# RuyiLian/CheckerPose

Hardware: AMD Instinct MI355X
Metric: crops/sec forward (256x256, npt=512) (higher is better)
Workload: dtype bf16; 1 GPU; LMO 'ape' hr18GNN2_res6_gnn3Skip_mlpQuery npt=512, PoseNet_GNNskip forward, deterministic random-init weights; global_batch=256, parallelism=dp1 (no forward collective), launch=hipGraph replay of 104 kernel launches

## Files before the change

### checkerpose_amd/_abi.py

```python
import ctypes as C
import os

_HERE = os.path.dirname(os.path.abspath(__file__))
LIB_PATH = os.environ.get("CHECKERPOSE_AMD_LIB") or os.path.join(_HERE, "libcheckerpose_hip.so")

CP_F32, CP_BF16, CP_F16 = 0, 1, 2
ACT_NONE, ACT_RELU, ACT_LEAKY = 0, 1, 2
LOSS_BCE, LOSS_L1 = 0, 1
POSE_ERR_ADD, POSE_ERR_ADI = 1, 2
BOP_ERR_MSSD, BOP_ERR_MSPD, BOP_ERR_PROJ, BOP_MAP_SMALL, BOP_MAP_LARGE = 1, 2, 4, 16, 32


class CpConvDesc(C.Structure):
    _fields_ = [("dtype", C.c_int32), ("out_f32", C.c_int32), ("B", C.c_int32), ("H", C.c_int32), ("W", C.c_int32),
                ("Cin", C.c_int32), ("in_cstride", C.c_int32), ("in_coff", C.c_int32),
                ("R", C.c_int32), ("S", C.c_int32), ("stride", C.c_int32), ("pad", C.c_int32),
                ("Ho", C.c_int32), ("Wo", C.c_int32), ("Cout", C.c_int32), ("act", C.c_int32), ("slope", C.c_float), ("ksplit", C.c_int32),
                ("o_base", C.c_int64), ("o_sb", C.c_int64), ("o_sy", C.c_int64), ("o_sx", C.c_int64),
                ("o_sc", C.c_int64)]


_P, _I, _F, _L = C.c_void_p, C.c_int, C.c_float, C.c_longlong


# ... 62 lines not shown
                ("Cin", C.c_int32), ("x_cstride", C.c_int32), ("x_coff", C.c_int32),
                ("R", C.c_int32), ("S", C.c_int32), ("stride", C.c_int32), ("pad", C.c_int32),
                ("dw_base", C.c_int64), ("dw_sco", C.c_int64), ("dw_sci", C.c_int64), ("dw_sr", C.c_int64),
                ("dw_ss", C.c_int64)]


SIGNATURES = {
    "cp_version": (_I, []),
    "cp_device_status": (_I, [_P, _I]),
    "cp_set_deterministic": (None, [_I]),
    "cp_get_deterministic": (_I, []),
    "cp_strerror": (C.c_char_p, [_I]),
    "cp_last_kernel": (C.c_char_p, []),
    "cp_kernel_log_begin": (None, []),
    "cp_kernel_log": (C.c_char_p, []),
    "cp_chan_align": (_I, [_I]),
    "cp_packed_weight_bytes": (C.c_size_t, [_I, _I, _I, _I, _I]),
    "cp_pack_conv_weight": (_I, [_P, _I, _P, _I, _I, _I, _I, _I, _I, _I, _P, _I, _P]),
    "cp_conv2d_igemm": (_I, [_P, C.POINTER(CpConvDesc), _P, _P, _P, _P, _P, _P]),
    "cp_conv2d_igemm_splitk": (_I, [_I, C.c_longlong, _I, _I]),
    "cp_packed_halo_weight_bytes": (C.c_size_t, [_I, _I, _I]),
    "cp_pack_conv3x3_halo_weight": (_I, [_P, _I, _P, _I, _I, _I, _P]),
    "cp_conv3x3_halo": (_I, [_P, C.POINTER(CpConvDesc), _P, _P, _P, _P, _P, _P]),
    "cp_conv2x2_halo_supported": (_I, [_I, _I, _I, _I]),
    "cp_packed_conv2x2_halo_weight_bytes": (C.c_size_t, [_I, _I, _I]),
    "cp_pack_conv2x2_halo_weight": (_I, [_P, _I, _P, _I, _I, _I, _P]),
    "cp_conv2x2_halo": (_I, [_P, C.POINTER(CpConvDesc), _P, _P, _P, _P, _P, _P]),
    "cp_conv3x3_s2_small_supported": (_I, [_I, _I, _I, _I]),
    "cp_conv3x3_s2_small_weight_bytes": (C.c_size_t, [_I, _I]),
    "cp_pack_conv3x3_s2_small_weight": (_I, [_P, _P, _I, _I, _I, _I, _P]),
    "cp_conv3x3_s2_small": (_I, [_P, C.POINTER(CpConvDesc), _P, _P, _P, _P, _P]),
    "cp_conv3x3_halo_up2x_supported": (_I, [_I, _I]),
    "cp_conv3x3_halo_up2x": (_I, [_P, C.POINTER(CpConvDesc), _P, _P, _P, _P, _P]),
    "cp_conv3x3_halo_seg_supported": (_I, [_I, _I, _I]),
    "cp_conv3x3_halo_seg": (_I, [_P, C.POINTER(CpConvDesc), _P, _P, _P, _P, _P, _P, _P, _I, _P]),
    "cp_pack_conv3x3_rows_weight": (_I, [_P, _I, _P, _I, _I, _I, _P]),
    "cp_basicblock_fused": (_I, [_P, C.POINTER(CpConvDesc), _P, _P, _P, _P, _P, _P, _P, _P]),
    "cp_bottleneck_fused": (_I, [_P, C.POINTER(CpConvDesc)] + [_P] * 14),
    "cp_packed_gemm_weight_bytes": (C.c_size_t, [_I, _I, _I]),
    "cp_pack_gemm_weight": (_I, [_P, _I, _P, _I, _I, _I, _P]),
    "cp_gemm_rows": (_I, [_P, C.POINTER(CpConvDesc), _P, _P, _P, _P, _P, _P]),
    "cp_mlp_query_fused_supported": (_I, [_I, _I, _I, _I]),
    "cp_mlp_query_fused": (_I, [_P, _P, _I, _I, _I, _I, _P, _P, _P, _F, _P, _P, _P, _F, _P, _P, _P, _L, _L, _L, _L]),
    "cp_mlp_query_fused_t": (_I, [_P, _I, _P, _I, _I, _I, _I, _P, _P, _P, _F, _P, _P, _P, _F, _P, _P, _P, _L, _L, _L, _L]),
    "cp_mlp_query_fused_n": (_I, [_P, _I, _P, _I, _I, _I, _I, _P, _P, _P, _F, _P, _P, _P, _F, _P, _P, _I, _P, _L, _L, _L, _L,
                                  _P, _P, _P, _P]),
    "cp_mlp_pair_fused_supported": (_I, [_I, _I, _I]),
    "cp_mlp_pair_fused": (_I, [_P, _P, _I, _I, _I, _I, _I, _P, _P, _F, _P, _P, _F, _P, _I, _I]),
    "cp_mlp_pair_fused_t": (_I, [_P, _I, _P, _I, _I, _I, _I, _I, _P, _P, _F, _P, _P, _F, _P, _I, _I]),
    "cp_mlp_pair_fused_gather_supported": (_I, [_I, _I, _I]),
    "cp_mlp_pair_fused_gather": (_I, [_P, C.POINTER(CpI2fGather), _P, _I, _I, _I, _I, _I, _P, _P, _F, _P, _P, _F, _P, _I, _I]),
    "cp_mlp_pair_fused_gather_t": (_I, [_P, _I, C.POINTER(CpI2fGather), _P, _I, _I, _I, _I, _I, _P, _P, _F, _P, _P, _F, _P, _I, _I]),
    "cp_hr_stem_weight_bytes": (C.c_size_t, [_I]),
    "cp_pack_hr_stem_weights": (_I, [_P, _P, _P, _P, _P]),
    "cp_hr_stem": (_I, [_P, _P, _I, _I, _I, _P, _P, _P, _P, _P, _P, _P]),
    "cp_hr_chain_supported": (_I, [_I, _I, _I]),
    "cp_hr_chain_weight_bytes": (C.c_size_t, [_I, _I, _I]),
    "cp_hr_chain_affine_floats": (_I, [_I, _I, _I]),
    "cp_pack_hr_chain_weight": (_I, [_P, _P, _P, _I, _I, _I, _I, _P]),
    "cp_hr_branch_chain": (_I, [_P, _I, _I, _I, _I, _I, C.POINTER(_P), C.POINTER(C.c_int32), _I, _P, _P, _P]),
    "cp_hr_chain_tail_supported": (_I, [_I, _I, _I]),
    "cp_hr_chain_tail_weight_bytes": (C.c_size_t, []),
    "cp_hr_chain_tail_channels": (_I, []),
    "cp_pack_hr_chain_tail_weight": (_I, [_P, _P, _P, _I, _I, _I, _P]),
    "cp_hr_branch_chain_tail": (_I, [_P, _I, _I, _I, _I, _I, C.POINTER(_P), C.POINTER(C.c_int32), _I, _P, _P, _P, C.POINTER(CpChainTail)]),
    "cp_hr_chain_tailconv_supported": (_I, [_I, _I, _I, _I, _I]),
# ... 175 lines not shown
```

### checkerpose_amd/engine.py

```python
import ctypes as C
import os

import torch

from . import _abi
from ._abi import ACT_LEAKY, ACT_NONE, ACT_RELU, CP_BF16, CP_F16, CP_F32, CpChainTail, CpChainTailConv, CpConvDesc, CpFuseConv

_TORCH_DT = {CP_F32: torch.float32, CP_BF16: torch.bfloat16}
USE_HALO = os.environ.get("CHECKERPOSE_AMD_HALO", "1") != "0"
USE_FUSED_BN = os.environ.get("CHECKERPOSE_AMD_FUSED_BN", "1") != "0"
USE_FUSED_BB = os.environ.get("CHECKERPOSE_AMD_FUSED_BB", "1") != "0"
USE_GEMM = os.environ.get("CHECKERPOSE_AMD_GEMM", "1") != "0"
USE_CHAIN = os.environ.get("CHECKERPOSE_AMD_CHAIN", "1") != "0"
USE_UP_FUSED = os.environ.get("CHECKERPOSE_AMD_UP_FUSED", "1") != "0"
USE_FUSE_OUT = os.environ.get("CHECKERPOSE_AMD_FUSE_OUT", "1") != "0"
USE_S2_SMALL = os.environ.get("CHECKERPOSE_AMD_S2_SMALL", "1") != "0"
USE_SEG_FUSED = os.environ.get("CHECKERPOSE_AMD_SEG_FUSED", "1") != "0"
USE_HALO2 = os.environ.get("CHECKERPOSE_AMD_HALO2", "1") != "0"
USE_CHAIN_TAILS = os.environ.get("CHECKERPOSE_AMD_CHAIN_TAILS", "1") != "0"
USE_CHAIN_TAIL = os.environ.get("CHECKERPOSE_AMD_CHAIN_TAIL", "1") != "0"
FUSE_OUT_MIN_BATCH = int(os.environ.get("CHECKERPOSE_AMD_FUSE_OUT_MIN_BATCH", "1"))
USE_MLP_FUSED = os.environ.get("CHECKERPOSE_AMD_MLP_FUSED", "1") != "0"
MLP_FUSED_MIN_ROWS = int(os.environ.get("CHECKERPOSE_AMD_MLP_FUSED_MIN_ROWS", "1"))
EDGE_SCHED = os.environ.get("CHECKERPOSE_AMD_EDGE_SCHED", "1") != "0"
USE_SPLITK = os.environ.get("CHECKERPOSE_AMD_SPLITK", "1") != "0"
GEMM_WS_SMALL_K = os.environ.get("CHECKERPOSE_AMD_GEMM_WS_SMALL_K", "1") != "0"
USE_MLP_GATHER = os.environ.get("CHECKERPOSE_AMD_MLP_GATHER", "1") != "0"
USE_PATCH_GATHER = os.environ.get("CHECKERPOSE_AMD_PATCH_GATHER", "1") != "0"
USE_STEM = os.environ.get("CHECKERPOSE_AMD_STEM", "1") != "0"
STEM_MIN_BATCH = int(os.environ.get("CHECKERPOSE_AMD_STEM_MIN_BATCH", "96"))
USE_EDGE_FUSED = os.environ.get("CHECKERPOSE_AMD_EDGE_FUSED", "1") != "0"
USE_GNN_F16 = os.environ.get("CHECKERPOSE_AMD_GNN_F16", "1") != "0"
USE_EDGE_TILED = os.environ.get("CHECKERPOSE_AMD_EDGE_TILED", "1") != "0"
EDGE_FUSED_MIN_BATCH = int(os.environ.get("CHECKERPOSE_AMD_EDGE_FUSED_MIN_BATCH", "96"))
CHAIN_MIN_BATCH = int(os.environ.get("CHECKERPOSE_AMD_CHAIN_MIN_BATCH", "40"))
NO_RECYCLE = os.environ.get("CHECKERPOSE_AMD_NO_RECYCLE", "0") == "1"
DTYPES = {"fp32": CP_F32, "f32": CP_F32, "float32": CP_F32, "bf16": CP_BF16, "bfloat16": CP_BF16}


class _ConvLog(list):

    def __init__(self, prog):
        super().__init__()
        self.prog, self.op_index = prog, []

    def append(self, e):
        super().append(e)
# ... 36 lines not shown
            raise RuntimeError("parameter %s must be an fp32 tensor on %s" % (key, self.device))
        return t.detach().contiguous()

    def pack(self, name, w, Cout, Cin, R, S, cin_phys, cout_rows, transposed=0, phase=0, row_map=None, dtype=None):
        dtype = self.dtype if dtype is None else dtype
        ck = (name, cin_phys, cout_rows, transposed, phase) + (() if dtype == self.dtype else (dtype,))
        if ck in self.cache:
            return self.cache[ck]
        nbytes = self.lib.cp_packed_weight_bytes(dtype, cout_rows, cin_phys, R, S)
        out = torch.empty(nbytes, dtype=torch.uint8, device=self.device)
        rm = None
        if row_map is not None:
            rm = torch.tensor(row_map, dtype=torch.int32, device=self.device)
            self.keep.append(rm)
        w = w.contiguous()
        self.keep.append(w)
        st = torch.cuda.current_stream(self.device).cuda_stream
        _abi.check(self.lib.cp_pack_conv_weight(st, dtype, w.data_ptr(), Cout, Cin, R, S, cin_phys, transposed, phase,
                                                rm.data_ptr() if rm is not None else None, cout_rows, out.data_ptr()),
                   "cp_pack_conv_weight(%s)" % name)
        self.cache[ck] = out
        return out

    def pack_halo(self, name, w, Cout, Cin, cin_phys):
        ck = ("halo", name, cin_phys)
        if ck in self.cache:
            return self.cache[ck]
        out = torch.empty(self.lib.cp_packed_halo_weight_bytes(self.dtype, Cout, cin_phys), dtype=torch.uint8, device=self.device)
        w = w.contiguous()
        self.keep.append(w)
        st = torch.cuda.current_stream(self.device).cuda_stream
        _abi.check(self.lib.cp_pack_conv3x3_halo_weight(st, self.dtype, w.data_ptr(), Cout, Cin, cin_phys, out.data_ptr()),
                   "cp_pack_conv3x3_halo_weight(%s)" % name)
        self.cache[ck] = out
        return out

    def pack_rows3x3(self, name, w, Cout, Cin, cin_phys):
        ck = ("rows3x3", name, cin_phys)
        if ck in self.cache:
            return self.cache[ck]
        out = torch.empty(self.lib.cp_packed_halo_weight_bytes(self.dtype, Cout, cin_phys), dtype=torch.uint8, device=self.device)
        w = w.contiguous()
        self.keep.append(w)
        st = torch.cuda.current_stream(self.device).cuda_stream
        _abi.check(self.lib.cp_pack_conv3x3_rows_weight(st, self.dtype, w.data_ptr(), Cout, Cin, cin_phys, out.data_ptr()),
                   "cp_pack_conv3x3_rows_weight(%s)" % name)
        self.cache[ck] = out
        return out

    def pack_gemm(self, name, w, Cout, Cin, cin_phys, dtype=None):
        dtype = self.dtype if dtype is None else dtype
        ck = ("gemm", name, cin_phys) + (() if dtype == self.dtype else (dtype,))
        if ck in self.cache:
            return self.cache[ck]
        out = torch.empty(self.lib.cp_packed_gemm_weight_bytes(dtype, Cout, cin_phys), dtype=torch.uint8, device=self.device)
        w = w.contiguous()
        self.keep.append(w)
        st = torch.cuda.current_stream(self.device).cuda_stream
        _abi.check(self.lib.cp_pack_gemm_weight(st, dtype, w.data_ptr(), Cout, Cin, cin_phys, out.data_ptr()),
                   "cp_pack_gemm_weight(%s)" % name)
        self.cache[ck] = out
        return out

    def pack_chain(self, name, ws, affs, C_, H, W):
        ck = ("chain", name)
        if ck in self.cache:
# ... 241 lines not shown

    def can_conv_up2x(self, H, W, Cout):
        return (USE_UP_FUSED and 2 * H >= 8 and 2 * W >= 16 and
                bool(self.lib.cp_conv3x3_halo_up2x_supported(self.dtype, _rup(Cout, self.E))))

    def conv_up2x(self, x: Act, wkey, w, scale, shift, act=ACT_NONE, slope=0.0, out: Act = None):
        wCout, wCin = w.shape[0], w.shape[1]
        if wCin != x.C:
            raise RuntimeError("conv %s: weight expects %d input channels, activation has %d" % (wkey, wCin, x.C))
        packed = self.ws.pack_halo(wkey, w, wCout, wCin, x.Cphys)
        sc, sh = self.ws.affine(wkey + "#0", scale, shift, wCout)
        Ho, Wo = 2 * x.H, 2 * x.W
        if out is None:
            out = self.act(Ho, Wo, wCout)
        d = CpConvDesc()
        d.dtype, d.out_f32 = self.dtype, 0
        d.B, d.H, d.W = x.B, Ho, Wo
        d.Cin, d.in_cstride, d.in_coff = x.Cphys, x.cstride, x.coff
        d.R, d.S, d.stride, d.pad, d.Ho, d.Wo = 3, 3, 1, 1, Ho, Wo
        d.act, d.slope, d.Cout = act, slope, out.Cphys
        d.o_base, d.o_sb, d.o_sy, d.o_sx, d.o_sc = out.coff, out.H * out.W * out.cstride, out.W * out.cstride, out.cstride, 1
        self.keep += [d, packed, sc, sh]
        fn = self.lib.cp_conv3x3_halo_up2x
        dref = C.byref(d)
        pw, ps, pt = packed.data_ptr(), sc.data_ptr(), sh.data_ptr()
        xtb, otb = x.tbuf, out.tbuf
        self._add(fn, lambda P: (dref, P(xtb), pw, ps, pt, P(otb)), "conv3x3_halo4:" + wkey, [xtb], [otb])
        fl = 2 * x.B * Ho * Wo * 9 * wCin * wCout
        self.flops += fl
        nbytes = x.B * x.H * x.W * wCin * self.es + x.B * Ho * Wo * wCout * self.es + 9 * wCin * wCout * self.es
        self.conv_log.append((wkey, x.B * Ho * Wo, wCout, 9 * wCin, fl, "conv3x3_halo4", nbytes))
        return out

    def can_conv_halo_seg(self, x: Act, Cout, S):
        return (USE_SEG_FUSED and USE_HALO and x.W >= 16 and x.H >= 8 and
                bool(self.lib.cp_conv3x3_halo_seg_supported(self.dtype, _rup(Cout, self.E), S)))

    def conv_halo_seg(self, x: Act, wkey, w, scale, shift, act, seg_key, seg_w, seg_b, seg_tbuf, slope=0.0):
        wCout, wCin = w.shape[0], w.shape[1]
        if wCin != x.C:
            raise RuntimeError("conv %s: weight expects %d input channels, activation has %d" % (wkey, wCin, x.C))
        packed = self.ws.pack_halo(wkey, w, wCout, wCin, x.Cphys)
        sc, sh = self.ws.affine(wkey + "#0", scale, shift, wCout)
        S = seg_w.shape[0]
        ck = ("seg_head", seg_key, self.dtype)
        if ck not in self.ws.cache:
            w2 = seg_w.reshape(S, wCout).float()
            if self.dtype == CP_BF16:
                w2 = w2.to(torch.bfloat16).float()
            self.ws.cache[ck] = (w2.contiguous().to(self.device), seg_b.float().contiguous().to(self.device))
        sw, sb = self.ws.cache[ck]
        out = self.act(x.H, x.W, wCout)
        d = CpConvDesc()
        d.dtype, d.out_f32 = self.dtype, 0
        d.B, d.H, d.W = x.B, x.H, x.W
        d.Cin, d.in_cstride, d.in_coff = x.Cphys, x.cstride, x.coff
        d.R, d.S, d.stride, d.pad, d.Ho, d.Wo = 3, 3, 1, 1, x.H, x.W
        d.act, d.slope, d.Cout = act, slope, out.Cphys
        d.o_base, d.o_sb, d.o_sy, d.o_sx, d.o_sc = out.coff, out.H * out.W * out.cstride, out.W * out.cstride, out.cstride, 1
        self.keep += [d, packed, sc, sh, sw, sb]
        fn = self.lib.cp_conv3x3_halo_seg
        dref = C.byref(d)
        pw, ps, pt, psw, psb = packed.data_ptr(), sc.data_ptr(), sh.data_ptr(), sw.data_ptr(), sb.data_ptr()
        xtb, otb = x.tbuf, out.tbuf
        self._add(fn, lambda P: (dref, P(xtb), pw, ps, pt, P(otb), psw, psb, S, P(seg_tbuf)), "conv3x3_halo4:" + wkey, [xtb], [otb, seg_tbuf])
        fl = 2 * x.B * x.H * x.W * 9 * wCin * wCout
# ... 793 lines not shown
```

### checkerpose_amd/netbuilder.py

```python
import os

import torch

from ._abi import ACT_LEAKY, ACT_NONE, ACT_RELU
from .engine import Act, Program, _rup

from .model.backbone import HRNET_CFGS
IMG_FEATS_DIMS = {"resnet34": [64, 128, 256, 512], "hrnet_w18": [128, 256, 512, 1024], "hrnet_w18_small": [128, 256, 512, 1024],
                  "hrnet_w30": [128, 256, 512, 1024]}


FUSE_OUT_DEEP = os.environ.get("CHECKERPOSE_AMD_FUSE_OUT_DEEP", "1") != "0"


DECODER_SPLITK = os.environ.get("CHECKERPOSE_AMD_DECODER_SPLITK", "1") != "0"
HEAD_ON_REFINE_LANE = os.environ.get("CHECKERPOSE_AMD_HEAD_LANE", "1") != "0"
FUSE_SAME_LANE = os.environ.get("CHECKERPOSE_AMD_FUSE_SAME_LANE", "1") != "0"


class NetEmitter:
    def __init__(self, prog: Program, sd):
        self.p, self.ws, self.sd = prog, prog.ws, sd
        self.ones = {}
        self.tp = prog if getattr(prog, "training", False) else None
# ... 628 lines not shown
        g = g()
        p.decode(dbits, -1, io["mask"], io["xid"], io["yid"], io["x64"], io["y64"], N)
        p.set_lane(0)
    cats = {}
    if tp is None:
        for i in range(1, active):
            if i in lowcats:
                continue
            sk = feats[-i - 1]
            cats[i] = p.act(2 * sk.H, 2 * sk.W, nf + sk.C)
            p.set_lane(2)
            p.upsample2x(sk, cats[i].slice(_rup(nf, p.E), sk.C))
    wseg = em.W("seg_block.weight")
    seg_fused = [False]

    def tail_conv(x, ck, bk, last, out=None):
        if (last and tp is None and out is None and p.can_conv_halo_seg(x, em.W(ck + ".weight").shape[0], wseg.shape[0])
                and not (DECODER_SPLITK and p.would_splitk(x.B * x.H * x.W, 9 * x.Cphys, em.W(ck + ".weight").shape[0]))):
            s_, t_ = em.ws.bn_fold(bk)
            seg_fused[0] = True
            return p.conv_halo_seg(x, ck, em.W(ck + ".weight"), s_, t_, ACT_RELU, "seg_block", wseg, em.W("seg_block.bias"), io["seg_tb"])
        return em.conv_bn(x, ck, bk, 3, 1, 1, out=out)

    for i in range(active):
        p.set_lane(0)
        up = "up_net.%d" % i
        last = i == active - 1
        if i == 0:
            wt = em.W(up + ".0.weight")
            s, t = em.ws.bn_fold(up + ".1") if tp is None else (None, None)
            o = p.act(2 * f.H, 2 * f.W, nf)
            if tp is not None:
                s, t = tp.const_vec(nf, True), tp.const_vec(nf, False)
            for ph in range(4):
                a, b = ph >> 1, ph & 1
                if tp is None and ph > 0:
                    p.set_lane(2 + ph)
                p.conv(f, up + ".0", wt, s, t, 1 + a, 1 + b, 1, 0, nf, ACT_RELU if tp is None else ACT_NONE, transposed=1, phase=ph,
                       ostr=((a * o.W + b) * o.cstride, o.H * o.W * o.cstride, 2 * o.W * o.cstride, 2 * o.cstride, 1),
                       out_tbuf=o.tbuf, out_hw=(f.H, f.W))
            if tp is None:
                p.set_lane(0)
                for ph in range(1, 4):
                    p.sync(2 + ph, 0)
            if tp is not None:
                o = _convt_train_tail(em, up, wt, f, o, nf)
            f = em.conv_bn(o, up + ".3", up + ".4", 3, 1, 1)
            f = tail_conv(f, up + ".6", up + ".7", last, out=lowcats[1].slice(0, nf) if 1 in lowcats else None)
        elif i in lowcats:
            s1, t1 = em.ws.bn_fold(up + ".2")
            f = p.conv_up2x(lowcats[i], up + ".1", em.W(up + ".1.weight"), s1, t1, ACT_RELU)
            f = tail_conv(f, up + ".4", up + ".5", last, out=lowcats[i + 1].slice(0, nf) if (i + 1) in lowcats else None)
        else:
            sk = feats[-i - 1]
            cat = cats[i] if i in cats else p.act(2 * f.H, 2 * f.W, f.C + sk.C)
            if i == 1 and i in cats:
                p.sync(2, 0)
            p.upsample2x(f, cat.slice(0, f.C))
            if i not in cats:
                p.upsample2x(sk, cat.slice(f.Cphys, sk.C))
            if tp is not None:
                _upsample_tape(tp, f, cat.slice(0, f.C))
                _upsample_tape(tp, sk, cat.slice(f.Cphys, sk.C))
            f = em.conv_bn(cat, up + ".1", up + ".2", 3, 1, 1)
            f = tail_conv(f, up + ".4", up + ".5", last, out=lowcats[i + 1].slice(0, nf) if (i + 1) in lowcats else None)
        p.sync(0, 1)
        p.set_lane(1)
        fdec = f
        if tp is None and cfg.get("export_dec"):
            p.to_nchw_f32(f, io["dec_feats"][i])
        if tp is None and cfg.get("inject_dec"):
            t_ = io["inject_dec"][i]
            f = p.nchw_to_nhwc(t_, t_.shape[1], t_.shape[2], t_.shape[3])
        rp = "refine_net.%d" % i
# ... 140 lines not shown

    p.set_lane(0)
    cats = {}
    if tp is None:
        for i in range(1, active):
            if i in lowcats:
                continue
            sk = feats[-i - 1]
            cats[i] = p.act(2 * sk.H, 2 * sk.W, nf + sk.C)
            p.set_lane(2)
            p.upsample2x(sk, cats[i].slice(_rup(nf, p.E), sk.C))
    wseg = em.W("seg_block.weight")
    seg_fused = False
    f = feats[-1]

    def tail_conv(x, ck, bk, last, out=None):
        nonlocal seg_fused
        if (last and tp is None and out is None and p.can_conv_halo_seg(x, em.W(ck + ".weight").shape[0], wseg.shape[0])
                and not (DECODER_SPLITK and p.would_splitk(x.B * x.H * x.W, 9 * x.Cphys, em.W(ck + ".weight").shape[0]))):
            s_, t_ = em.ws.bn_fold(bk)
            seg_fused = True
            return p.conv_halo_seg(x, ck, em.W(ck + ".weight"), s_, t_, ACT_RELU, "seg_block", wseg, em.W("seg_block.bias"), io["seg_tb"])
        return em.conv_bn(x, ck, bk, 3, 1, 1, out=out)

    for i in range(active):
        p.set_lane(0)
        up = "up_net.%d" % i
        last = i == active - 1
        nxt = lowcats[i + 1].slice(0, nf) if (i + 1) in lowcats else None
        if i == 0:
            wt = em.W(up + ".0.weight")
            s, t = em.ws.bn_fold(up + ".1") if tp is None else (tp.const_vec(nf, True), tp.const_vec(nf, False))
            o = p.act(2 * f.H, 2 * f.W, nf)
            for ph in range(4):
                a, b = ph >> 1, ph & 1
                if tp is None and ph > 0:
                    p.set_lane(2 + ph)
                p.conv(f, up + ".0", wt, s, t, 1 + a, 1 + b, 1, 0, nf, ACT_RELU if tp is None else ACT_NONE, transposed=1, phase=ph,
                       ostr=((a * o.W + b) * o.cstride, o.H * o.W * o.cstride, 2 * o.W * o.cstride, 2 * o.cstride, 1),
                       out_tbuf=o.tbuf, out_hw=(f.H, f.W))
            if tp is None:
                p.set_lane(0)
                for ph in range(1, 4):
                    p.sync(2 + ph, 0)
            else:
                o = _convt_train_tail(em, up, wt, f, o, nf)
            f = em.conv_bn(o, up + ".3", up + ".4", 3, 1, 1)
            f = tail_conv(f, up + ".6", up + ".7", last, out=nxt)
        elif i in lowcats:
            s1, t1 = em.ws.bn_fold(up + ".2")
            f = p.conv_up2x(lowcats[i], up + ".1", em.W(up + ".1.weight"), s1, t1, ACT_RELU)
            f = tail_conv(f, up + ".4", up + ".5", last, out=nxt)
        else:
            sk = feats[-i - 1]
            cat = cats[i] if i in cats else p.act(2 * f.H, 2 * f.W, f.C + sk.C)
            if i == 1 and i in cats:
                p.sync(2, 0)
            p.upsample2x(f, cat.slice(0, f.C))
            if i not in cats:
                p.upsample2x(sk, cat.slice(f.Cphys, sk.C))
            if tp is not None:
                _upsample_tape(tp, f, cat.slice(0, f.C))
                _upsample_tape(tp, sk, cat.slice(f.Cphys, sk.C))
            f = em.conv_bn(cat, up + ".1", up + ".2", 3, 1, 1)
            f = tail_conv(f, up + ".4", up + ".5", last, out=nxt)
    sd_ = wseg.shape[0]
    if seg_fused:
        pass
    elif tp is None:
        p.conv(f, "seg_block", wseg, em._unit(sd_), em.W("seg_block.bias"), 1, 1, 1, 0, sd_, out_f32=True,
               ostr=(0, sd_ * f.H * f.W, f.W, 1, f.H * f.W), out_tbuf=io["seg_tb"])
    else:
        p.conv(f, "seg_block", wseg, tp.const_vec(sd_, True), em._bias_vec("seg_block", sd_), 1, 1, 1, 0, sd_, out_f32=True,
               ostr=(0, sd_ * f.H * f.W, f.W, 1, f.H * f.W), out_tbuf=io["seg_tb"])
        em._out_layer_bwd("seg_block", wseg, f, sd_, io["dseg"], 0, sd_ * f.H * f.W, 1, f.H * f.W)
    p.par_end()
    return feats, f
```

### include/checkerpose_hip.h

```cpp
#ifndef CHECKERPOSE_HIP_H
#define CHECKERPOSE_HIP_H

#include <stddef.h>
#include <stdint.h>

#ifdef __cplusplus
extern "C" {
#endif

typedef void* cp_stream_t;

enum { CP_F32 = 0, CP_BF16 = 1, CP_F16 = 2 };
enum { CP_ACT_NONE = 0, CP_ACT_RELU = 1, CP_ACT_LEAKY = 2 };
enum { CP_LOSS_BCE = 0, CP_LOSS_L1 = 1 };
enum {
  CP_OK = 0,
  CP_ERR_INVALID = -1,
  CP_ERR_HIP = -2,
  CP_ERR_ALIGN = -3,
  CP_ERR_RANGE = -4
};

int cp_version(void);
const char* cp_strerror(int code);
// ... 18 lines not shown
  int32_t dtype;
  int32_t out_f32;
  int32_t B, H, W;
  int32_t Cin;
  int32_t in_cstride;
  int32_t in_coff;
  int32_t R, S, stride, pad;
  int32_t Ho, Wo;
  int32_t Cout;
  int32_t act;
  float slope;
  int32_t ksplit;
  int64_t o_base, o_sb, o_sy, o_sx, o_sc;
} CpConvDesc;

int cp_conv2d_igemm(cp_stream_t stream, const CpConvDesc* d, const void* in, const void* packed_w,
                    const float* scale, const float* shift, const void* residual, void* out);
int cp_conv2d_igemm_splitk(int dtype, long long M, int K, int Cout);

size_t cp_packed_halo_weight_bytes(int dtype, int Cout, int cin_phys);
int cp_pack_conv3x3_halo_weight(cp_stream_t stream, int dtype, const float* w, int Cout, int Cin, int cin_phys,
                                void* packed);
int cp_conv3x3_halo(cp_stream_t stream, const CpConvDesc* d, const void* in, const void* packed_w,
                    const float* scale, const float* shift, const void* residual, void* out);
int cp_conv2x2_halo_supported(int dtype, int H, int W, int Cout_phys);
size_t cp_packed_conv2x2_halo_weight_bytes(int dtype, int Cout, int Cin_phys);
int cp_pack_conv2x2_halo_weight(cp_stream_t stream, int dtype, const float* w, int Cout, int Cin, int cin_phys, void* packed);
int cp_conv2x2_halo(cp_stream_t stream, const CpConvDesc* d, const void* in, const void* packed_w, const float* scale,
                    const float* shift, const void* residual, void* out);

int cp_conv3x3_halo_up2x_supported(int dtype, int Cout);
int cp_conv3x3_halo_up2x(cp_stream_t stream, const CpConvDesc* d, const void* in, const void* packed_w,
                         const float* scale, const float* shift, void* out);

int cp_conv3x3_halo_seg_supported(int dtype, int Cout, int S);
int cp_conv3x3_halo_seg(cp_stream_t stream, const CpConvDesc* d, const void* in, const void* packed_w, const float* scale,
                        const float* shift, void* out, const float* seg_w, const float* seg_b, int S, float* seg_out);

int cp_conv3x3_s2_small_supported(int H, int W, int cin_phys, int out_cphys);
size_t cp_conv3x3_s2_small_weight_bytes(int cin_phys, int out_cphys);
int cp_pack_conv3x3_s2_small_weight(cp_stream_t stream, const float* w, int Cout, int Cin, int cin_phys, int out_cphys, void* packed);
int cp_conv3x3_s2_small(cp_stream_t stream, const CpConvDesc* d, const void* in, const void* packed_w, const float* scale,
                        const float* shift, void* out);

int cp_pack_conv3x3_rows_weight(cp_stream_t stream, int dtype, const float* w, int Cout, int Cin, int cin_phys,
                                void* packed);
int cp_basicblock_fused(cp_stream_t stream, const CpConvDesc* d, const void* in, const void* packed_w1,
                        const float* scale1, const float* shift1, const void* packed_w2, const float* scale2,
                        const float* shift2, void* out);

int cp_bottleneck_fused(cp_stream_t stream, const CpConvDesc* d, const void* in, const void* packed_w1,
                        const float* scale1, const float* shift1, const void* packed_w2, const float* scale2,
                        const float* shift2, const void* packed_w3, const float* scale3, const float* shift3,
                        const void* packed_wd, const float* scaled, const float* shiftd, void* out);

size_t cp_packed_gemm_weight_bytes(int dtype, int Cout, int cin_phys);
int cp_pack_gemm_weight(cp_stream_t stream, int dtype, const float* w, int Cout, int Cin, int cin_phys, void* packed);
int cp_gemm_rows(cp_stream_t stream, const CpConvDesc* d, const void* in, const void* packed_w,
                 const float* scale, const float* shift, const void* residual, void* out);

int cp_mlp_query_fused_supported(int C0, int C1, int C2, int C3);
int cp_mlp_query_fused(cp_stream_t stream, const void* in, int in_cstride, int in_coff, int B, int N,
                       const void* packed_w1, const float* scale1, const float* shift1, float slope1,
                       const void* packed_w2, const float* scale2, const float* shift2, float slope2,
                       const float* w3, const float* b3, float* out, long long o_base, long long o_sb, long long o_sn, long long o_sc);
int cp_mlp_query_fused_t(cp_stream_t stream, int dtype, const void* in, int in_cstride, int in_coff, int B, int N,
// ... 400 lines not shown
```

Measured before the change: 25620 crops/s.

## Fuse four transposed-conv phases into one halo-staged MFMA kernel

Adds a kernel that computes all four output phases of the stride-2 3x3 transposed convolution in a single launch. It stages an input tile with a one-pixel halo in LDS and reuses each A fragment across the phases that share a tap. This replaces four per-phase implicit-GEMM launches plus their multi-lane syncs, cutting launch count, repeated input reads and cross-stream synchronisation. In exchange the four phases now run serially inside one kernel instead of concurrently on separate lanes. Occupancy may suffer because each thread holds a large 4x8 accumulator array.

```diff
diff --git a/checkerpose_amd/_abi.py b/checkerpose_amd/_abi.py
--- a/checkerpose_amd/_abi.py
+++ b/checkerpose_amd/_abi.py
@@ -118,6 +118,10 @@
     "cp_conv3x3_s2_small": (_I, [_P, C.POINTER(CpConvDesc), _P, _P, _P, _P, _P]),
     "cp_conv3x3_halo_up2x_supported": (_I, [_I, _I]),
     "cp_conv3x3_halo_up2x": (_I, [_P, C.POINTER(CpConvDesc), _P, _P, _P, _P, _P]),
+    "cp_convt3x3_s2_fused_supported": (_I, [_I, _I, _I, _I, _I]),
+    "cp_packed_convt_weight_bytes": (C.c_size_t, [_I, _I, _I]),
+    "cp_pack_convt_weight": (_I, [_P, _I, _P, _I, _I, _I, _P]),
+    "cp_convt3x3_s2_fused": (_I, [_P, C.POINTER(CpConvDesc), _P, _P, _P, _P, _P]),
     "cp_conv3x3_halo_seg_supported": (_I, [_I, _I, _I]),
     "cp_conv3x3_halo_seg": (_I, [_P, C.POINTER(CpConvDesc), _P, _P, _P, _P, _P, _P, _P, _I, _P]),
     "cp_pack_conv3x3_rows_weight": (_I, [_P, _I, _P, _I, _I, _I, _P]),
diff --git a/checkerpose_amd/csrc/convt_s2.hip b/checkerpose_amd/csrc/convt_s2.hip
--- /dev/null
+++ b/checkerpose_amd/csrc/convt_s2.hip
@@ -0,0 +1,276 @@
+#include <stdlib.h>
+
+#include "common.h"
+
+struct ConvtParams {
+  const void* in; const void* w; const float* scale; const float* shift; void* out;
+  int B, H, W, Cin, in_cs, in_coff, nchunk, NB;
+  int G, TR, P, FR, FC, bands, total_tiles, plane;
+  int act; float slope;
+  uint32_t in_bytes, w_bytes;
+  long long o_base, o_sb, o_sy, o_sx;
+};
+
+template <typename Tag> struct MmaCt;
+template <> struct MmaCt<F32Tag> {
+  static __device__ __forceinline__ void run(const u32x4& w, const u32x4& a, f32x4& acc) {
+    acc = __builtin_amdgcn_mfma_f32_16x16x4f32(__uint_as_float(w.x), __uint_as_float(a.x), acc, 0, 0, 0);
+    acc = __builtin_amdgcn_mfma_f32_16x16x4f32(__uint_as_float(w.y), __uint_as_float(a.y), acc, 0, 0, 0);
+    acc = __builtin_amdgcn_mfma_f32_16x16x4f32(__uint_as_float(w.z), __uint_as_float(a.z), acc, 0, 0, 0);
+    acc = __builtin_amdgcn_mfma_f32_16x16x4f32(__uint_as_float(w.w), __uint_as_float(a.w), acc, 0, 0, 0);
+  }
+};
+template <> struct MmaCt<BF16Tag> {
+  static __device__ __forceinline__ void run(const u32x4& w, const u32x4& a, f32x4& acc) {
+    acc = __builtin_amdgcn_mfma_f32_16x16x32_bf16(__builtin_bit_cast(bf16x8, w), __builtin_bit_cast(bf16x8, a), acc, 0, 0, 0);
+  }
+};
+
+constexpr int CT_NF = 8;
+constexpr int CT_MAXSLOT = 256;
+
+static __device__ __forceinline__ bool ct_frag(const ConvtParams& p, int f, int& j, int& y, int& col0) {
+  int R0;
+  if (p.FC == 1) { R0 = f * p.FR; col0 = 0; } else { R0 = f / p.FC; col0 = 16 * (f - R0 * p.FC); }
+  j = R0 / p.TR; y = R0 - j * p.TR;
+  return j < p.G;
+}
+
+template <typename Tag>
+__global__ __launch_bounds__(256, 2) void convt3x3_s2_fused_kernel(const ConvtParams p) {
+  constexpr int E = Tag::E;
+  constexpr int KCH = 4 * E;
+  constexpr int ES = 16 / E;
+  extern __shared__ __attribute__((aligned(16))) unsigned char smem[];
+  const int HB = 4 * p.plane;
+
+  const int label = blockIdx.x & 7, slot = blockIdx.x >> 3;
+  const int nblk = slot % p.NB;
+  const int t = label * ((p.total_tiles + 7) >> 3) + slot / p.NB;
+  if (t >= p.total_tiles) return;
+  const int grp = t / p.bands, band = t - grp * p.bands;
+  const int b0 = grp * p.G, y0 = band * p.TR;
+
+  const int tid = threadIdx.x;
+  const int lane = tid & 63;
+  const int wave = __builtin_amdgcn_readfirstlane(tid >> 6);
+  const int x = lane & 15, q = lane >> 4;
+  const int g = nblk * 4 + wave;
+
+  const __amdgpu_buffer_rsrc_t rsrc = __builtin_amdgcn_make_buffer_rsrc(const_cast<void*>(p.in), 0, p.in_bytes, 0x00020000);
+  const __amdgpu_buffer_rsrc_t wrsrc = __builtin_amdgcn_make_buffer_rsrc(const_cast<void*>(p.w), 0, p.w_bytes, 0x00020000);
+
+  const int W1 = p.W + 1, cropsz = (p.TR + 1) * W1, nstage = p.G * cropsz;
+  uint32_t s_goff[4], s_lds[4];
+#pragma unroll
+  for (int k = 0; k < 4; ++k) {
+    const int i = tid + 256 * k;
+    const int hp = i >> 2, pq = i & 3;
+    const int j = hp / cropsz, rem = hp - j * cropsz;
+    const int py = rem / W1, px = rem - py * W1;
+    const int b = b0 + j, gy = y0 + py;
+    const bool in_tile = hp < nstage;
+    const bool ok = in_tile & (b < p.B) & (gy < p.H) & (px < p.W);
+    s_goff[k] = ok ? (uint32_t)(((b * p.H + gy) * p.W + px) * p.in_cs + p.in_coff + pq * E) : 0xFFFFFFFFu;
+    s_lds[k] = in_tile ? (uint32_t)(pq * p.plane + ((j * (p.TR + 1) + py) * p.P + px) * 16) : 0xFFFFFFFFu;
+  }
+  const int s_cq = (tid & 3) * E;
+  auto stage_load = [&](u32x4* v, int c) {
+    const int c0 = c * KCH;
+#pragma unroll
+    for (int k = 0; k < 4; ++k) {
+      const bool ok = (s_goff[k] != 0xFFFFFFFFu) & (c0 + s_cq < p.Cin);
+      v[k] = __builtin_bit_cast(u32x4, __builtin_amdgcn_raw_buffer_load_b128(rsrc, ok ? (s_goff[k] + (uint32_t)c0) * ES : 0x80000000u, 0, 0));
+    }
+  };
+  auto stage_write = [&](const u32x4* v, int buf) {
+#pragma unroll
+    for (int k = 0; k < 4; ++k)
+      if (s_lds[k] != 0xFFFFFFFFu) *(u32x4*)(smem + buf * HB + s_lds[k]) = v[k];
+  };
+
+  uint32_t f_off[CT_NF];
+#pragma unroll
+  for (int f = 0; f < CT_NF; ++f) {
+    int j, y, col0;
+    const bool v = ct_frag(p, f, j, y, col0);
+    f_off[f] = v ? (uint32_t)(((j * (p.TR + 1) + y) * p.P + col0) * 16) : 0u;
+  }
+  const int lrow = p.FC == 1 && p.W < 16 ? x / p.W : 0;
+  const int lcol = p.FC == 1 && p.W < 16 ? x - lrow * p.W : x;
+  const uint32_t a_lane = (uint32_t)(q * p.plane + (lrow * p.P + lcol) * 16);
+  auto a_load = [&](u32x4* a, int buf, int r, int s, int half) {
+    const unsigned char* base = smem + buf * HB + a_lane + (r * p.P + s) * 16;
+#pragma unroll
+    for (int i = 0; i < 4; ++i) a[i] = *(const u32x4*)(base + f_off[4 * half + i]);
+  };
+
+  f32x4 acc[4][CT_NF];
+#pragma unroll
+  for (int ph = 0; ph < 4; ++ph)
+#pragma unroll
+    for (int f = 0; f < CT_NF; ++f) acc[ph][f] = f32x4{0.f, 0.f, 0.f, 0.f};
+
+  const uint32_t wbase = ((uint32_t)g * p.nchunk * 9u * 64u + lane) * 16u;
+  auto w_load = [&](u32x4* w, int c, int first, int n) {
+    const uint32_t off = wbase + ((uint32_t)c * 9u + (uint32_t)first) * 1024u;
+#pragma unroll
+    for (int i = 0; i < 4; ++i)
+      if (i < n) w[i] = __builtin_bit_cast(u32x4, __builtin_amdgcn_raw_buffer_load_b128(wrsrc, off + i * 1024u, 0, 0));
+  };
+
+  u32x4 sv[4];
+  u32x4 w0[4], w1[2], w2[2], w3[1], a0[4], a1[4];
+  stage_load(sv, 0);
+  w_load(w0, 0, 0, 4); w_load(w1, 0, 4, 2); w_load(w2, 0, 6, 2); w_load(w3, 0, 8, 1);
+  stage_write(sv, 0);
+  __syncthreads();
+
+#define CT_MMA(AF, HALF, WS, NB_, P0, P1, P2, P3)                                                     \
+  { constexpr int ph_[4] = {P0, P1, P2, P3};                                                          \
+    _Pragma("unroll") for (int i_ = 0; i_ < 4; ++i_)                                                  \
+      _Pragma("unroll") for (int n_ = 0; n_ < NB_; ++n_) MmaCt<Tag>::run(WS[n_], AF[i_], acc[ph_[n_]][4 * HALF + i_]); }
+#define CT_TAP(R, S, RN, SN, LAST, WS, FIRST, NB_, P0, P1, P2, P3)                                    \
+  a_load(a1, buf, R, S, 1); __builtin_amdgcn_sched_barrier(0);                                        \
+  CT_MMA(a0, 0, WS, NB_, P0, P1, P2, P3) __builtin_amdgcn_sched_barrier(0);                           \
+  if (!LAST) a_load(a0, buf, RN, SN, 0);                                                              \
+  __builtin_amdgcn_sched_barrier(0);                                                                  \
+  CT_MMA(a1, 1, WS, NB_, P0, P1, P2, P3) __builtin_amdgcn_sched_barrier(0);                           \
+  w_load(WS, c + 1, FIRST, NB_);
+  for (int c = 0; c < p.nchunk; ++c) {
+    const int buf = c & 1;
+    stage_load(sv, c + 1);
+    a_load(a0, buf, 0, 0, 0);
+    CT_TAP(0, 0, 0, 1, false, w0, 0, 4, 0, 1, 2, 3)
+    CT_TAP(0, 1, 1, 0, false, w1, 4, 2, 1, 3, 0, 0)
+    CT_TAP(1, 0, 1, 1, false, w2, 6, 2, 2, 3, 0, 0)
+    CT_TAP(1, 1, 0, 0, true, w3, 8, 1, 3, 0, 0, 0)
+    stage_write(sv, buf ^ 1);
+    __syncthreads();
+  }
+#undef CT_TAP
+#undef CT_MMA
+
+  const int ch = g * 16 + q * 4;
+  const f32x4 sc = *(const f32x4*)(p.scale + ch), sh = *(const f32x4*)(p.shift + ch);
+  const float sl = cp_act_slope(p.act, p.slope);
+#pragma unroll
+  for (int f = 0; f < CT_NF; ++f) {
+    int j, y, col0;
+    const bool v = ct_frag(p, f, j, y, col0);
+    const int b = b0 + j, sy = y0 + y + lrow, sx = col0 + lcol;
+    if (!(v && b < p.B && sy < p.H && sx < p.W)) continue;
+#pragma unroll
+    for (int ph = 0; ph < 4; ++ph) {
+      const long long o = p.o_base + (long long)b * p.o_sb + (long long)(2 * sy + (ph >> 1)) * p.o_sy + (long long)(2 * sx + (ph & 1)) * p.o_sx + ch;
+      float r[4];
+#pragma unroll
+      for (int k = 0; k < 4; ++k) r[k] = cp_act_apply(acc[ph][f][k] * sc[k] + sh[k], sl);
+      if (E == 4) *(f32x4*)((float*)p.out + o) = f32x4{r[0], r[1], r[2], r[3]};
+      else *(u32x2*)((uint16_t*)p.out + o) = u32x2{pack_bf16x2(r[0], r[1]), pack_bf16x2(r[2], r[3])};
+    }
+  }
+}
+
+template <typename Tag>
+__global__ void pack_convt_weight_kernel(const float* __restrict__ w, void* __restrict__ out, int Cout, int Cin, int nchunk, size_t total) {
+  constexpr int E = Tag::E;
+  const size_t i = (size_t)blockIdx.x * blockDim.x + threadIdx.x;
+  if (i >= total) return;
+  const int e = (int)(i % E);
+  const int lane = (int)((i / E) % 64);
+  size_t blk = i / (E * 64);
+  const int k = (int)(blk % 9); blk /= 9;
+  const int c = (int)(blk % nchunk);
+  const int g = (int)(blk / nchunk);
+  const int tap = k < 4 ? 0 : (k < 6 ? 1 : (k < 8 ? 2 : 3));
+  const int ph = k < 4 ? k : (k == 4 ? 1 : (k == 6 ? 2 : 3));
+  const int r = tap >> 1, s = tap & 1, a = ph >> 1, b = ph & 1;
+  const int kh = a ? (r ? 0 : 2) : 1, kw = b ? (s ? 0 : 2) : 1;
+  const int n = g * 16 + (lane & 15);
+  const int cin = c * (4 * E) + (lane >> 4) * E + e;
+  float v = 0.f;
+  if (n < Cout && cin < Cin) v = w[(((size_t)cin * Cout + n) * 3 + kh) * 3 + kw];
+  store_elem<Tag>(out, i, v);
+}
+
+static bool convt_geom(int H, int W, ConvtParams* p) {
+  if (H <= 0 || W < 4 || W > 64) return false;
+  int RB;
+  if (W < 16) {
+    if (16 % W) return false;
+    p->FR = 16 / W; p->FC = 1; RB = CT_NF * p->FR;
+    if (H % p->FR) return false;
+    p->P = W == 8 ? 24 : 12;
+  } else {
+    if (W % 16) return false;
+    p->FR = 1; p->FC = W / 16; RB = CT_NF / p->FC;
+    p->P = W + 1;
+  }
+  if (H <= RB) { p->TR = H; p->G = RB / H; p->bands = 1; }
+  else { p->TR = RB; p->G = 1; p->bands = (H + RB - 1) / RB; }
+  const int nslot = p->G * (p->TR + 1) * p->P;
+  p->plane = ((nslot + 15) / 16) * 256;
+  if (p->G * (p->TR + 1) * (W + 1) > CT_MAXSLOT) return false;
+  return 8 * p->plane <= 65536;
+}
+
+extern "C" int cp_convt3x3_s2_fused_supported(int dtype, int H, int W, int cin_phys, int cout_phys) {
+  ConvtParams p;
+  return (dtype == CP_F32 || dtype == CP_BF16) && cin_phys > 0 && cin_phys % 32 == 0 && cout_phys > 0 && cout_phys % 64 == 0 &&
+         (long long)H * W <= 64 * 64 && convt_geom(H, W, &p) ? 1 : 0;
+}
+
+extern "C" size_t cp_packed_convt_weight_bytes(int dtype, int Cout, int cin_phys) {
+  const int KCH = 4 * cp_chan_align(dtype);
+  return (((size_t)Cout + 15) / 16) * (((size_t)cin_phys + KCH - 1) / KCH) * 9 * 1024;
+}
+
+extern "C" int cp_pack_convt_weight(cp_stream_t stream, int dtype, const float* w, int Cout, int Cin, int cin_phys, void* packed) {
+  if (!w || !packed || Cout <= 0 || Cin <= 0 || cin_phys < Cin) return CP_ERR_INVALID;
+  if (dtype != CP_F32 && dtype != CP_BF16) return CP_ERR_INVALID;
+  const int E = cp_chan_align(dtype);
+  if (cin_phys % E || !cp_aligned16(packed)) return CP_ERR_ALIGN;
+  const int nchunk = (cin_phys + 4 * E - 1) / (4 * E);
+  const size_t total = cp_packed_convt_weight_bytes(dtype, Cout, cin_phys) / cp_elem_size(dtype);
+  const unsigned blocks = (unsigned)((total + 255) / 256);
+  if (dtype == CP_F32)
+    CP_LAUNCH(pack_convt_weight_kernel<F32Tag>, dim3(blocks), dim3(256), 0, (hipStream_t)stream, w, packed, Cout, Cin, nchunk, total);
+  else
+    CP_LAUNCH(pack_convt_weight_kernel<BF16Tag>, dim3(blocks), dim3(256), 0, (hipStream_t)stream, w, packed, Cout, Cin, nchunk, total);
+  return cp_check_launch();
+}
+
+extern "C" int cp_convt3x3_s2_fused(cp_stream_t stream, const CpConvDesc* d, const void* in, const void* packed_w, const float* scale,
+                                    const float* shift, void* out) {
+  if (!d || !in || !packed_w || !scale || !shift || !out) return CP_ERR_INVALID;
+  if (!cp_act_ok(d->act, d->slope) || d->B <= 0 || d->out_f32 || d->o_sc != 1) return CP_ERR_INVALID;
+  if (d->R != 3 || d->S != 3 || d->stride != 2 || d->pad != 1 || d->Ho != 2 * d->H || d->Wo != 2 * d->W) return CP_ERR_INVALID;
+  if (!cp_convt3x3_s2_fused_supported(d->dtype, d->H, d->W, d->Cin, d->Cout)) return CP_ERR_INVALID;
+  const int E = cp_chan_align(d->dtype), es = cp_elem_size(d->dtype);
+  if (d->in_coff % E || d->in_cstride % E || d->in_coff + d->Cin > d->in_cstride) return CP_ERR_ALIGN;
+  if (!cp_aligned16(in) || !cp_aligned16(packed_w) || !cp_aligned16(scale) || !cp_aligned16(shift) || !cp_aligned16(out)) return CP_ERR_ALIGN;
+  if ((d->o_base % 4) || (d->o_sb % 4) || (d->o_sy % 4) || (d->o_sx % 4)) return CP_ERR_ALIGN;
+  const long long in_bytes = (long long)d->B * d->H * d->W * d->in_cstride * es;
+  if (in_bytes >= (1LL << 31)) return CP_ERR_RANGE;
+  ConvtParams p;
+  convt_geom(d->H, d->W, &p);
+  p.in = in; p.w = packed_w; p.scale = scale; p.shift = shift; p.out = out;
+  p.B = d->B; p.H = d->H; p.W = d->W; p.Cin = d->Cin; p.in_cs = d->in_cstride; p.in_coff = d->in_coff;
+  p.nchunk = d->Cin / (4 * E);
+  p.NB = d->Cout / 64;
+  const long long tt = (long long)((d->B + p.G - 1) / p.G) * p.bands;
+  if (tt >= (1LL << 28)) return CP_ERR_RANGE;
+  p.total_tiles = (int)tt;
+  p.act = d->act; p.slope = d->slope;
+  p.in_bytes = (uint32_t)in_bytes;
+  const size_t wb = cp_packed_convt_weight_bytes(d->dtype, d->Cout, d->Cin);
+  if (wb >= (1ull << 31)) return CP_ERR_RANGE;
+  p.w_bytes = (uint32_t)wb;
+  p.o_base = d->o_base; p.o_sb = d->o_sb; p.o_sy = d->o_sy; p.o_sx = d->o_sx;
+  const unsigned grid = (unsigned)(((tt + 7) / 8) * 8 * p.NB);
+  const size_t lds = (size_t)8 * p.plane;
+  if (d->dtype == CP_F32) CP_LAUNCH(convt3x3_s2_fused_kernel<F32Tag>, dim3(grid), dim3(256), lds, (hipStream_t)stream, p);
+  else CP_LAUNCH(convt3x3_s2_fused_kernel<BF16Tag>, dim3(grid), dim3(256), lds, (hipStream_t)stream, p);
+  return cp_check_launch();
+}
diff --git a/checkerpose_amd/engine.py b/checkerpose_amd/engine.py
--- a/checkerpose_amd/engine.py
+++ b/checkerpose_amd/engine.py
@@ -13,6 +13,7 @@
 USE_GEMM = os.environ.get("CHECKERPOSE_AMD_GEMM", "1") != "0"
 USE_CHAIN = os.environ.get("CHECKERPOSE_AMD_CHAIN", "1") != "0"
 USE_UP_FUSED = os.environ.get("CHECKERPOSE_AMD_UP_FUSED", "1") != "0"
+USE_CONVT_FUSED = os.environ.get("CHECKERPOSE_AMD_CONVT_FUSED", "1") != "0"
 USE_FUSE_OUT = os.environ.get("CHECKERPOSE_AMD_FUSE_OUT", "1") != "0"
 USE_S2_SMALL = os.environ.get("CHECKERPOSE_AMD_S2_SMALL", "1") != "0"
 USE_SEG_FUSED = os.environ.get("CHECKERPOSE_AMD_SEG_FUSED", "1") != "0"
@@ -115,6 +116,19 @@
         st = torch.cuda.current_stream(self.device).cuda_stream
         _abi.check(self.lib.cp_pack_conv3x3_halo_weight(st, self.dtype, w.data_ptr(), Cout, Cin, cin_phys, out.data_ptr()),
                    "cp_pack_conv3x3_halo_weight(%s)" % name)
+        self.cache[ck] = out
+        return out
+
+    def pack_convt(self, name, w, Cout, Cin, cin_phys):
+        ck = ("convt", name, cin_phys)
+        if ck in self.cache:
+            return self.cache[ck]
+        out = torch.empty(self.lib.cp_packed_convt_weight_bytes(self.dtype, Cout, cin_phys), dtype=torch.uint8, device=self.device)
+        w = w.contiguous()
+        self.keep.append(w)
+        st = torch.cuda.current_stream(self.device).cuda_stream
+        _abi.check(self.lib.cp_pack_convt_weight(st, self.dtype, w.data_ptr(), Cout, Cin, cin_phys, out.data_ptr()),
+                   "cp_pack_convt_weight(%s)" % name)
         self.cache[ck] = out
         return out
 
@@ -422,6 +436,41 @@
         self.conv_log.append((wkey, x.B * Ho * Wo, wCout, 9 * wCin, fl, "conv3x3_halo4", nbytes))
         return out
 
+    def can_convt_fused(self, x: Act, Cout):
+        if not USE_CONVT_FUSED or self.ws.repacks_every_step or self.dtype not in (CP_F32, CP_BF16):
+            return False
+        if any(self.would_splitk(x.B * x.H * x.W, (1 + a) * (1 + b) * x.Cphys, Cout) for a in (0, 1) for b in (0, 1)):
+            return False
+        return bool(self.lib.cp_convt3x3_s2_fused_supported(self.dtype, x.H, x.W, x.Cphys, _rup(Cout, self.E)))
+
+    def convt_fused(self, x: Act, wkey, w, scale, shift, act=ACT_NONE, slope=0.0, out: Act = None):
+        wCin, wCout = w.shape[0], w.shape[1]
+        if wCin != x.C:
+            raise RuntimeError("conv %s: weight expects %d input channels, activation has %d" % (wkey, wCin, x.C))
+        packed = self.ws.pack_convt(wkey, w, wCout, wCin, x.Cphys)
+        sc, sh = self.ws.affine(wkey + "#fused", scale, shift, wCout)
+        Ho, Wo = 2 * x.H, 2 * x.W
+        if out is None:
+            out = self.act(Ho, Wo, wCout)
+        d = CpConvDesc()
+        d.dtype, d.out_f32 = self.dtype, 0
+        d.B, d.H, d.W = x.B, x.H, x.W
+        d.Cin, d.in_cstride, d.in_coff = x.Cphys, x.cstride, x.coff
+        d.R, d.S, d.stride, d.pad, d.Ho, d.Wo = 3, 3, 2, 1, Ho, Wo
+        d.act, d.slope, d.Cout = act, slope, _rup(wCout, self.E)
+        d.o_base, d.o_sb, d.o_sy, d.o_sx, d.o_sc = out.coff, out.H * out.W * out.cstride, out.W * out.cstride, out.cstride, 1
+        self.keep += [d, packed, sc, sh]
+        fn = self.lib.cp_convt3x3_s2_fused
+        dref = C.byref(d)
+        pw, ps, pt = packed.data_ptr(), sc.data_ptr(), sh.data_ptr()
+        xtb, otb = x.tbuf, out.tbuf
+        self._add(fn, lambda P: (dref, P(xtb), pw, ps, pt, P(otb)), "conv_igemm:" + wkey, [xtb], [otb])
+        fl = 2 * x.B * x.H * x.W * 9 * wCin * wCout
+        self.flops += fl
+        nbytes = x.B * x.H * x.W * wCin * self.es + x.B * Ho * Wo * wCout * self.es + 9 * wCin * wCout * self.es
+        self.conv_log.append((wkey, x.B * x.H * x.W, 4 * wCout, 4 * wCin, fl, "conv_igemm", nbytes))
+        return out
+
     def can_conv_halo_seg(self, x: Act, Cout, S):
         return (USE_SEG_FUSED and USE_HALO and x.W >= 16 and x.H >= 8 and
                 bool(self.lib.cp_conv3x3_halo_seg_supported(self.dtype, _rup(Cout, self.E), S)))
diff --git a/checkerpose_amd/netbuilder.py b/checkerpose_amd/netbuilder.py
--- a/checkerpose_amd/netbuilder.py
+++ b/checkerpose_amd/netbuilder.py
@@ -684,14 +684,17 @@
             o = p.act(2 * f.H, 2 * f.W, nf)
             if tp is not None:
                 s, t = tp.const_vec(nf, True), tp.const_vec(nf, False)
-            for ph in range(4):
+            fused = tp is None and p.can_convt_fused(f, nf)
+            if fused:
+                p.convt_fused(f, up + ".0", wt, s, t, ACT_RELU, out=o)
+            for ph in range(0 if fused else 4):
                 a, b = ph >> 1, ph & 1
                 if tp is None and ph > 0:
                     p.set_lane(2 + ph)
                 p.conv(f, up + ".0", wt, s, t, 1 + a, 1 + b, 1, 0, nf, ACT_RELU if tp is None else ACT_NONE, transposed=1, phase=ph,
                        ostr=((a * o.W + b) * o.cstride, o.H * o.W * o.cstride, 2 * o.W * o.cstride, 2 * o.cstride, 1),
                        out_tbuf=o.tbuf, out_hw=(f.H, f.W))
-            if tp is None:
+            if tp is None and not fused:
                 p.set_lane(0)
                 for ph in range(1, 4):
                     p.sync(2 + ph, 0)
@@ -898,18 +901,21 @@
             wt = em.W(up + ".0.weight")
             s, t = em.ws.bn_fold(up + ".1") if tp is None else (tp.const_vec(nf, True), tp.const_vec(nf, False))
             o = p.act(2 * f.H, 2 * f.W, nf)
-            for ph in range(4):
+            fused = tp is None and p.can_convt_fused(f, nf)
+            if fused:
+                p.convt_fused(f, up + ".0", wt, s, t, ACT_RELU, out=o)
+            for ph in range(0 if fused else 4):
                 a, b = ph >> 1, ph & 1
                 if tp is None and ph > 0:
                     p.set_lane(2 + ph)
                 p.conv(f, up + ".0", wt, s, t, 1 + a, 1 + b, 1, 0, nf, ACT_RELU if tp is None else ACT_NONE, transposed=1, phase=ph,
                        ostr=((a * o.W + b) * o.cstride, o.H * o.W * o.cstride, 2 * o.W * o.cstride, 2 * o.cstride, 1),
                        out_tbuf=o.tbuf, out_hw=(f.H, f.W))
-            if tp is None:
+            if tp is None and not fused:
                 p.set_lane(0)
                 for ph in range(1, 4):
                     p.sync(2 + ph, 0)
-            else:
+            elif tp is not None:
                 o = _convt_train_tail(em, up, wt, f, o, nf)
             f = em.conv_bn(o, up + ".3", up + ".4", 3, 1, 1)
             f = tail_conv(f, up + ".6", up + ".7", last, out=nxt)
diff --git a/include/checkerpose_hip.h b/include/checkerpose_hip.h
--- a/include/checkerpose_hip.h
+++ b/include/checkerpose_hip.h
@@ -74,6 +74,12 @@
 int cp_conv3x3_halo_up2x_supported(int dtype, int Cout);
 int cp_conv3x3_halo_up2x(cp_stream_t stream, const CpConvDesc* d, const void* in, const void* packed_w,
                          const float* scale, const float* shift, void* out);
+
+int cp_convt3x3_s2_fused_supported(int dtype, int H, int W, int cin_phys, int cout_phys);
+size_t cp_packed_convt_weight_bytes(int dtype, int Cout, int cin_phys);
+int cp_pack_convt_weight(cp_stream_t stream, int dtype, const float* w, int Cout, int Cin, int cin_phys, void* packed);
+int cp_convt3x3_s2_fused(cp_stream_t stream, const CpConvDesc* d, const void* in, const void* packed_w, const float* scale,
+                         const float* shift, void* out);
 
 int cp_conv3x3_halo_seg_supported(int dtype, int Cout, int S);
 int cp_conv3x3_halo_seg(cp_stream_t stream, const CpConvDesc* d, const void* in, const void* packed_w, const float* scale,
```

New measurement: 25890 crops/s (median of 4 runs). No clear change (+1.1%).
